# at-wat/mcl_3dl

Measured on AMD Instinct MI355X. Metric: particle·point evals/sec; filter-update Hz @ 4096 particles × 16k-pt scan, higher is better.
Workload: dtype f32

## Files before the change

### mcl_3dl_amd/csrc/host_measure.h

```cpp
#pragma once
#include <type_traits>

namespace
{
int ensure_structures(mcl3dl_hip_ctx* ctx, bool need_lik, bool need_dda, bool need_cells = false)
{
  if (!ctx->has_map)
    return ctx->fail(-5, "no map: call mcl3dl_hip_set_map first");
  bool built = false;
  if (need_lik && ctx->opt.lik_index == 0 && !need_cells && !ctx->lik_params_set && (ctx->lik_cell_from_beam || lik_cell_is_beams(ctx)))
  {
    ctx->lik_params_set = true;
    if (ctx->lik_cell_from_beam)
      ctx->lik_dirty = ctx->lik_base_dirty = true;
  }
  if (need_lik && (ctx->opt.lik_index == 0 || need_cells) && ctx->lik_dirty)
  {
    TRY(build_lik_grid(ctx));
    built = true;
  }
  if (need_lik && ctx->opt.lik_index == 0 && !need_cells)
  {
    const int dim[3] = { ctx->lg.nx, ctx->lg.ny, ctx->lg.nz };
    if (!lik_scan_provable(dim))
// ... 26 lines not shown
  k.r2_sq = static_cast<float>(static_cast<double>(r2) * static_cast<double>(r2));
  const double cell = 1.0 / static_cast<double>(ctx->lg.inv_cell);
  const auto reach = [&](float r) { return static_cast<int>(std::min(std::ceil(static_cast<double>(r) / cell + 0.005), 1.0e6)); };
  k.reach1 = reach(r1);
  k.reach2 = reach(r2);
  k.wx = ctx->weight[0];
  k.wy = ctx->weight[1];
  k.wz = ctx->weight[2];
  k.has_weight = ctx->has_weight ? 1 : 0;
  k.map = ctx->map_dev.as<float4>();
  k.occ = ctx->kd_occ.as<uint32_t>();
  return k;
}

int ensure_caster_structures(mcl3dl_hip_ctx* ctx, bool need_lik, bool need_beam, bool need_cells = false)
{
  if (ctx->beam_raycast != 1)
    return ensure_structures(ctx, need_lik, need_beam, need_cells);
  TRY(ensure_structures(ctx, need_lik, false, need_cells));
  if (need_beam)
  {
    if (ctx->lik_dirty)
    {
      TRY(build_lik_grid(ctx));
      scratch_trim(ctx, 64u << 20);
    }
    TRY(ensure_map_dev(ctx));
    const KdRayParams k = kd_ray_params(ctx);
    if (ctx->kd_occ_reach != k.reach1)
    {
      const unsigned long long n_cells = static_cast<unsigned long long>(ctx->lg.nx) * ctx->lg.ny * ctx->lg.nz;
      const unsigned long long blocks = (n_cells + 255) / 256;
      if (blocks > 0x7fffffffull)
        return ctx->fail(-4, "the cell grid has too many cells for the kd-tree caster's occupancy bitmap");
      TRY(ensure(ctx, ctx->kd_occ, sizeof(unsigned long long) * ((n_cells + 63) / 64)));
      hipLaunchKernelGGL(kd_occupancy_kernel, dim3(static_cast<unsigned>(blocks)), dim3(256), 0, ctx->stream, ctx->lg, k.reach1,
                         n_cells, ctx->kd_occ.as<unsigned long long>());
      HIP_TRY(hipGetLastError());
      ctx->kd_occ_reach = k.reach1;
    }
  }
  return 0;
}

using HostOut = PfEmit;

LikParams lik_params(const mcl3dl_hip_ctx* ctx)
{
  LikParams p;
  p.wx = ctx->weight[0];
  p.wy = ctx->weight[1];
  p.wz = ctx->weight[2];
  p.has_weight = ctx->has_weight ? 1 : 0;
  p.match_dist_min = ctx->match_dist_min;
  p.r2 = static_cast<float>(static_cast<double>(ctx->match_dist_min) * static_cast<double>(ctx->match_dist_min));
  p.match_dist_flat = ctx->match_dist_flat;
  p.match_weight = ctx->match_weight;
  return p;
}

BeamParams beam_params(const mcl3dl_hip_ctx* ctx)
{
  BeamParams p;
  p.sin_total_ref = ctx->sin_total_ref;
  p.hit_range_sq = ctx->hit_range_sq;
  p.filter_label_max = ctx->filter_label_max;
  p.short_only = ctx->short_only;
  p.beam_likelihood_min = ctx->beam_likelihood_min;
  return p;
}

void beam_refresh(mcl3dl_hip_ctx* ctx)
{
  ctx->hit_range_sq = static_cast<float>(std::pow(static_cast<double>(ctx->hit_range), 2));
  ctx->beam_likelihood = static_cast<float>(
      std::pow(static_cast<double>(ctx->beam_likelihood_min), 1.0 / static_cast<float>(ctx->beam_num_points)));
  ctx->sin_total_ref = sinf(ctx->ang_total_ref);
  ctx->pow_table_dirty = true;
}

uint64_t morton3(uint32_t x, uint32_t y, uint32_t z)
{
  auto spread = [](uint64_t v)
  {
    v &= 0x1fffff;
    v = (v | v << 32) & 0x1f00000000ffffULL;
    v = (v | v << 16) & 0x1f0000ff0000ffULL;
    v = (v | v << 8) & 0x100f00f00f00f00fULL;
    v = (v | v << 4) & 0x10c30c30c30c30c3ULL;
    v = (v | v << 2) & 0x1249249249249249ULL;
    return v;
  };
  return spread(x) | (spread(y) << 1) | (spread(z) << 2);
}

int ensure_pow_table(mcl3dl_hip_ctx* ctx, size_t n_b_coming = 0)
{
  const size_t n_b = std::max(ctx->n_b, n_b_coming);
  if (!(ctx->pow_table_dirty || n_b > ctx->pow_table_len))
    return 0;
  const size_t len = std::max<size_t>(n_b, 1024);
  std::vector<float> table(len + 1);
  table[0] = 1.0f;
  for (size_t k = 1; k <= len; ++k)
    table[k] = table[k - 1] * ctx->beam_likelihood;
  TRY(ensure(ctx, ctx->pow_table, sizeof(float) * table.size()));
// ... 969 lines not shown
```

### mcl_3dl_amd/csrc/likelihood_kernels.h

```cpp
#pragma once
#include <hip/hip_runtime.h>
#include <stdint.h>

#include "device_math.h"
#include "float_chain.h"
#include "map_structs.h"
#pragma clang fp contract(off)

namespace mcl3dl
{
template <bool STATS>
__device__ inline float nearest_d2(const LikGrid& g, float qx, float qy, float qz, unsigned& n_tested)
{
  const float fx = floorf((qx - g.ox) * g.inv_cell);
  const float fy = floorf((qy - g.oy) * g.inv_cell);
  const float fz = floorf((qz - g.oz) * g.inv_cell);
  float best = 3.0e38f;
  if (!(fx >= 1.0f && fy >= 1.0f && fz >= 1.0f && fx <= static_cast<float>(g.nx - 2) &&
        fy <= static_cast<float>(g.ny - 2) && fz <= static_cast<float>(g.nz - 2)))
    return best;
  const int cx = static_cast<int>(fx), cy = static_cast<int>(fy), cz = static_cast<int>(fz);
  uint32_t rs[9], re[9];
#pragma unroll
  for (int r = 0; r < 9; ++r)
  {
    const int dz = r / 3 - 1, dy = r % 3 - 1;
    const size_t row = (static_cast<size_t>(cz + dz) * g.ny + (cy + dy)) * g.nx + cx;
    rs[r] = g.cell_start[row - 1];
    re[r] = g.cell_start[row + 2];
  }
#pragma unroll
  for (int r = 0; r < 9; ++r)
  {
    for (uint32_t k = rs[r]; k < re[r]; ++k)
    {
      const float4 p = g.pts[k];
      const float dx = qx - p.x, dy = qy - p.y, dz = qz - p.z;
      float d2 = dx * dx;
      d2 = d2 + dy * dy;
      d2 = d2 + dz * dz;
      best = d2 < best ? d2 : best;
      if (STATS)
        ++n_tested;
    }
  }
  return best;
}

__device__ inline float d2_simple(float qx, float qy, float qz, float px, float py, float pz)
{
  const float dx = qx - px, dy = qy - py, dz = qz - pz;
  float d2 = dx * dx;
  d2 = d2 + dy * dy;
  d2 = d2 + dz * dz;
  return d2;
}

__global__ void radius_search_kernel(const float* __restrict__ query_xyz, int n, LikGrid g, LikParams prm, float radius,
                                     float r2, int reach, int* __restrict__ out_index, float* __restrict__ out_sqdist)
// ... 552 lines not shown
  {
    __shared__ float s_small[256];
    const int row = static_cast<int>(threadIdx.x) - i;
    if (i < n_s)
      s_small[row + static_cast<int>(perm[i])] = term;
    __syncthreads();
    float s = 0.0f;
    if (i == 0)
      for (int j = 0; j < n_s; ++j)
        s = s + s_small[row + j];
    lik = s;
  }
  else
  {
    double acc = static_cast<double>(term);
#pragma unroll
    for (int off = W / 2; off > 0; off >>= 1)
      acc += __shfl_down(acc, off, W);
    lik = static_cast<float>(acc);
  }
#pragma unroll
  for (int off = W / 2; off > 0; off >>= 1)
    num += __shfl_down(num, off, W);
  if (i == 0 && p < n_p)
  {
    if (out_lik)
      out_lik[p] = lik;
    if (out_ratio)
      out_ratio[p] = static_cast<float>(num) / static_cast<float>(n_s);
  }
}

struct LikChain
{
  unsigned long long* carry;
  uint32_t tag0;
  float* out_lik;
  float* out_ratio;
  float* also_fill;
  volatile unsigned* err;
};

__device__ inline unsigned long long chain_pack(uint32_t value, uint32_t tag)
{
  return (static_cast<unsigned long long>(tag) << 32) | value;
}

template <bool B>
struct BoolConstant
{
  static constexpr bool value = B;
};

constexpr int DEFER_QCAP = 96;

struct DeferQueue
{
  uint32_t word[4][DEFER_QCAP];
  uint16_t who[4][DEFER_QCAP];
};

template <bool FAST = false>
__device__ inline float eval_coop_first(const RecGrid& rg, const LikParams& prm, const Vec3f pos, const Quat rot, const float4 v,
                                        bool have_point, int lane, bool& matched, bool& over, float& best, uint32_t& mine,
                                        unsigned long long& over_m, unsigned long long* matched_m = nullptr)
{
  const Vec3f tp = vadd(qrot_trim(rot, Vec3f{ v.x, v.y, v.z }), pos);
  const float qx = tp.x * prm.wx, qy = tp.y * prm.wy, qz = tp.z * prm.wz;
  uint32_t ti, sub;
  const bool inside = rec_locate<FAST>(rg, qx, qy, qz, ti, sub) && have_point;
  int b;
  if constexpr (FAST)
  {
    const unsigned long long base = reinterpret_cast<unsigned long long>(rg.brick_table);
    const u32x4 tb = { static_cast<uint32_t>(base), (static_cast<uint32_t>(base >> 32) & 0xffffu) | (4u << 16), rg.table_bytes32,
                       0x00020000u };
    asm volatile("buffer_load_dword %0, %1, %2, 0 idxen\n\ts_waitcnt vmcnt(0)" : "=v"(b) : "v"(inside ? ti : rg.ti_empty), "s"(tb) : "memory");
  }
  else
    b = rg.brick_table[inside ? ti : rg.ti_empty];
  const bool valid = b >= 0;
  float dist = -1.0f;
  over = false;
  over_m = 0ull;
  best = 0.0f;
  mine = 0u;
  const unsigned long long valid_m = __builtin_amdgcn_ballot_w64(valid);
  if (valid_m != 0ull)
  {
    if constexpr (FAST)
      asm("" : "+v"(sub));
    uint32_t rec = (static_cast<uint32_t>(b) << 9) | sub;
    if constexpr (FAST)
      asm("" : "+v"(rec));
    const uint32_t vrec = (FAST || rg.rec_bytes32) ? rec : (valid ? rec : 0u);
    uint32_t w[4];
    best = quad_round<FAST>(rg.rec, rg.rec_bytes32, vrec, qx, qy, qz, lane & 3, w);
    mine = own_word(w, lane & 3);
    over_m = valid_m & lanes_gt_u32(mine, rg.over_thr);
    if (rg.bound_step > 0.0f && over_m != 0ull)
    {
      asm volatile("");
      over_m &= __builtin_amdgcn_fcmpf(best, rec_bound2(rg, mine), 2 );
    }
    over = __builtin_amdgcn_inverse_ballot_w64(over_m);
    if constexpr (FAST)
    {
      const unsigned long long in_m = valid_m & ~over_m & __builtin_amdgcn_fcmpf(best, prm.r2, 4 );
      float out = over ? best : 0.0f * prm.match_weight;
      if (__builtin_amdgcn_inverse_ballot_w64(in_m))
        out = lik_dist(prm, sqrt_in_radius(best)) * prm.match_weight;
      *matched_m = in_m;
      matched = __builtin_amdgcn_inverse_ballot_w64(in_m);
      return out;
    }
    if (valid && !over && best < prm.r2)
    {
      const float s = sqrt_in_radius(best);
      dist = lik_dist(prm, s);
    }
  }
  if constexpr (FAST)
  {
    *matched_m = 0ull;
    matched = false;
    return 0.0f * prm.match_weight;
  }
  matched = !(dist < 0.0f);
  return lik_term(prm, dist, matched);
}

template <bool FAST = false, int G, int LD>
__device__ inline void defer_drain(const RecGrid& rg, const LikParams& prm, const float (&s_pose)[G][8], float (&s_term)[G][LD],
                                   unsigned (&s_cnt)[G][4], const DeferQueue& q, int wave, int lane, uint32_t base, uint32_t n,
                                   const float4 v)
{
  __builtin_amdgcn_fence(__ATOMIC_RELEASE, "wavefront");
  __builtin_amdgcn_wave_barrier();
  const bool act = static_cast<uint32_t>(lane) < n;
  const uint32_t slot = act ? base + static_cast<uint32_t>(lane) : base;
  const uint32_t word = q.word[wave][slot];
  const uint32_t who = q.who[wave][slot];
  const int src = static_cast<int>(who & 63u), k = static_cast<int>(who >> 6);
  const Vec3f pt = { __shfl(v.x, src), __shfl(v.y, src), __shfl(v.z, src) };
  const Vec3f pos = { s_pose[k][0], s_pose[k][1], s_pose[k][2] };
  const Quat rot = { s_pose[k][3], s_pose[k][4], s_pose[k][5], s_pose[k][6] };
  const Vec3f tp = vadd(qrot_trim(rot, pt), pos);
  const float qx = tp.x * prm.wx, qy = tp.y * prm.wy, qz = tp.z * prm.wz;
  const int t_src = wave * 64 + src;
  float best = s_term[k][t_src];
  const uint32_t ext = word & rec_ext_mask(rg);
  const uint32_t rounds = act ? rec_overflow_records(word >> rg.count_shift, 4u, rg.count_is_records) : 0u;
  for (uint32_t r = 0; wave_any(r < rounds); ++r)
  {
    const bool more = r < rounds;
    uint32_t unused[4];
    const float m = quad_round<FAST>(rg.ovf, rg.ovf_bytes32, more ? ext + r : 0u, qx, qy, qz, lane & 3, unused);
    best = (more && m < best) ? m : best;
  }
  if constexpr (FAST)
  {
    if (act)
    {
      const bool in = best < prm.r2;
      s_term[k][t_src] = in ? lik_dist(prm, sqrt_in_radius(best)) * prm.match_weight : 0.0f * prm.match_weight;
      if (in)
        atomicAdd(&s_cnt[k][wave], 1u);
    }
    return;
  }
  float dist = -1.0f;
  if (act && best < prm.r2)
  {
    const float s = sqrt_in_radius(best);
    dist = lik_dist(prm, s);
  }
  if (act)
  {
    s_term[k][t_src] = lik_term(prm, dist, !(dist < 0.0f));
    if (!(dist < 0.0f))
      atomicAdd(&s_cnt[k][wave], 1u);
  }
}

template <bool FAST, int G, int LD>
__device__ __forceinline__ uint32_t defer_push(const RecGrid& rg, const LikParams& prm, const float (&s_pose)[G][8],
                                               float (&s_term)[G][LD], unsigned (&s_cnt)[G][4], DeferQueue& q, int wave, int lane,
                                               const float4 v, uint32_t qn, unsigned long long over_m, bool over, uint32_t mine,
                                               int k)
{
  if (over_m != 0ull)
  {
    const uint32_t n_new = static_cast<uint32_t>(__popcll(over_m));
    if (qn + n_new > static_cast<uint32_t>(DEFER_QCAP))
    {
      defer_drain<FAST>(rg, prm, s_pose, s_term, s_cnt, q, wave, lane, 0u, qn, v);
      qn = 0;
    }
    if (over)
    {
      const uint32_t slot = qn + __builtin_amdgcn_mbcnt_hi(static_cast<uint32_t>(over_m >> 32),
                                                           __builtin_amdgcn_mbcnt_lo(static_cast<uint32_t>(over_m), 0u));
      q.word[wave][slot] = mine;
      q.who[wave][slot] = static_cast<uint16_t>((static_cast<uint32_t>(k) << 6) | static_cast<uint32_t>(lane));
    }
    qn += n_new;
    if (qn >= 64u)
    {
      defer_drain<FAST>(rg, prm, s_pose, s_term, s_cnt, q, wave, lane, qn - 64u, 64u, v);
      qn -= 64u;
    }
  }
  return qn;
}

template <bool FAST, int G, int LD>
__device__ __forceinline__ void defer_flush(const RecGrid& rg, const LikParams& prm, const float (&s_pose)[G][8],
                                            float (&s_term)[G][LD], unsigned (&s_cnt)[G][4], const DeferQueue& q, int wave,
                                            int lane, const float4 v, uint32_t qn)
{
  defer_drain<FAST>(rg, prm, s_pose, s_term, s_cnt, q, wave, lane, 0u, qn, v);
}

template <int G>
__device__ __forceinline__ void stage_poses(float (&s_pose)[G][8], const float* __restrict__ pose7, int n_p, int group, int t)
{
  if (t < G)
  {
    const int p = group * G + t;
    float valid = 0.f;
    if (p < n_p)
    {
      const float* ps = pose7 + 7 * static_cast<size_t>(p);
      const Quat r = qnormalized(Quat{ ps[3], ps[4], ps[5], ps[6] });
      s_pose[t][0] = ps[0];
      s_pose[t][1] = ps[1];
      s_pose[t][2] = ps[2];
      s_pose[t][3] = r.x;
      s_pose[t][4] = r.y;
      s_pose[t][5] = r.z;
      s_pose[t][6] = r.w;
      valid = 1.f;
    }
    s_pose[t][7] = valid;
  }
}

__device__ __forceinline__ bool xcd_row_map(uint32_t block_index, int n_groups, int n_links, int& link, int& group)
{
  const uint32_t xcd = block_index & 7u, seq = block_index >> 3, ng = static_cast<uint32_t>(n_groups);
  const uint32_t row = seq / ng;
  link = static_cast<int>(row * 8u + xcd);
  group = static_cast<int>(seq - row * ng);
  return link < n_links;
}

constexpr int CHAIN_POLL_MAX = 1 << 20;
__device__ __forceinline__ void chain_take(const LikChain& ch, const unsigned long long* cw, int link, float& s,
                                           uint32_t& cnt)
{
  s = 0.0f;
  cnt = 0;
  if (link > 0)
  {
    const uint32_t want = ch.tag0 + static_cast<uint32_t>(link) - 1u;
    unsigned long long a = 0, b = 0;
#pragma nounroll
    for (int polls = 0;; ++polls)
    {
      a = __hip_atomic_load(cw, __ATOMIC_RELAXED, __HIP_MEMORY_SCOPE_AGENT);
      b = __hip_atomic_load(cw + 1, __ATOMIC_RELAXED, __HIP_MEMORY_SCOPE_AGENT);
      if (static_cast<uint32_t>(a >> 32) == want && static_cast<uint32_t>(b >> 32) == want)
        break;
      if (polls >= CHAIN_POLL_MAX)
// ... 33 lines not shown
    if (ch.also_fill)
      ch.also_fill[p] = 1.0f;
  }
  else
  {
    const uint32_t tag = ch.tag0 + static_cast<uint32_t>(link);
    __hip_atomic_store(cw, chain_pack(__float_as_uint(s), tag), __ATOMIC_RELAXED, __HIP_MEMORY_SCOPE_AGENT);
    __hip_atomic_store(cw + 1, chain_pack(cnt, tag), __ATOMIC_RELAXED, __HIP_MEMORY_SCOPE_AGENT);
  }
}

template <int G, int MODE, int MINW = 8, bool COOP = false, bool DEFER = false, bool CHAIN = false>
__device__ __forceinline__ void likelihood_tiled_body(const uint32_t block_index, const float* __restrict__ pose7, int n_p,
                                                      const float4* __restrict__ scan, int n_s, int n_tiles, int n_groups,
                                                      LikGrid g, RecGrid rg, LikParams prm,
                                                      double* __restrict__ partial_sum, unsigned* __restrict__ partial_cnt,
                                                      const uint32_t* __restrict__ scan_perm, float* __restrict__ strict_terms,
                                                      int strict_skew4, LikChain ch)
{
  constexpr int TERM_LD = CHAIN ? 260 : 256;
  __shared__ __attribute__((aligned(16))) float s_pose[G][8];
  __shared__ __attribute__((aligned(16))) float s_term[G][TERM_LD];
  __shared__ unsigned s_cnt[G][4];
  const uint32_t xcd = block_index & 7u;
  const uint32_t seq = block_index >> 3;
  const uint32_t ng = static_cast<uint32_t>(n_groups);
  const uint32_t full_tiles = static_cast<uint32_t>(n_tiles) & ~7u;
  const uint32_t per_xcd_full = (full_tiles >> 3) * ng;
  int tile, group;
  if constexpr (CHAIN)
  {
    if (!xcd_row_map(block_index, n_groups, n_tiles, tile, group))
      return;
  }
  else if (seq < per_xcd_full)
  {
    const uint32_t row = seq / ng;
    tile = static_cast<int>(row * 8u + xcd);
    group = static_cast<int>(seq - row * ng);
  }
  else
  {
    const uint32_t rem_items = (static_cast<uint32_t>(n_tiles) - full_tiles) * ng;
    const uint32_t per_xcd_rem = (rem_items + 7u) >> 3;
    const uint32_t s2 = seq - per_xcd_full;
    const uint32_t item = xcd * per_xcd_rem + s2;
    if (s2 >= per_xcd_rem || item >= rem_items)
      return;
    const uint32_t row = item / ng;
    tile = static_cast<int>(full_tiles + row);
    group = static_cast<int>(item - row * ng);
  }
  const int t = threadIdx.x, lane = t & 63, wave = t >> 6;
  stage_poses<G>(s_pose, pose7, n_p, group, t);
  const int i = tile * 256 + t;
  const bool have_point = i < n_s;
  const float4 v = have_point ? scan[i] : make_float4(0.f, 0.f, 0.f, 0.f);
  __syncthreads();
  const int n_valid = min(G, n_p - group * G);
  if constexpr (COOP && MODE == 2 && DEFER)
  {
    __shared__ DeferQueue s_q;
    const auto pose_loop = [&](auto fast) {
      constexpr bool FAST = decltype(fast)::value;
      uint32_t qn = 0;
      typedef float f32x4 __attribute__((ext_vector_type(4)));
      typedef __attribute__((address_space(3))) const f32x4 LdsPose;
      typedef __attribute__((address_space(3))) float LdsTerm;
      typedef __attribute__((address_space(3))) unsigned LdsCount;
      LdsPose* p_pose = (LdsPose*)&s_pose[0][0];
      LdsTerm* p_term = (LdsTerm*)&s_term[0][t];
      LdsCount* p_cnt = (LdsCount*)&s_cnt[0][wave];
      for (int k = 0; k < n_valid; ++k)
      {
        LdsPose* ps = FAST ? p_pose : (LdsPose*)&s_pose[k][0];
        const f32x4 pa = ps[0], pb = ps[1];
        const Vec3f pos = { pa.x, pa.y, pa.z };
        const Quat rot = { pa.w, pb.x, pb.y, pb.z };
        bool matched, over;
        float best;
        uint32_t mine;
        unsigned long long om;
        unsigned long long m;
        if constexpr (FAST)
        {
          *p_term = eval_coop_first<true>(rg, prm, pos, rot, v, have_point, lane, matched, over, best, mine, om, &m);
          if (lane == 0)
            *p_cnt = static_cast<unsigned>(__popcll(m));
          asm volatile("" : "+v"(p_pose), "+v"(p_term), "+v"(p_cnt));
          p_pose += 2;
          p_term += TERM_LD;
          p_cnt += 4;
        }
        else
        {
          const float term = eval_coop_first(rg, prm, pos, rot, v, have_point, lane, matched, over, best, mine, om);
          s_term[k][t] = over ? best : term;
          m = __builtin_amdgcn_ballot_w64(matched);
          if (lane == 0)
            s_cnt[k][wave] = static_cast<unsigned>(__popcll(m));
        }
        qn = defer_push<FAST>(rg, prm, s_pose, s_term, s_cnt, s_q, wave, lane, v, qn, om, over, mine, k);
      }
      if (qn != 0u)
        defer_flush<FAST>(rg, prm, s_pose, s_term, s_cnt, s_q, wave, lane, v, qn);
    };
    if (rg.common_map)
      pose_loop(BoolConstant<true>{});
    else
      pose_loop(BoolConstant<false>{});
  }
  else if constexpr (COOP && MODE == 2)
  {
    for (int k = 0; k < n_valid; ++k)
    {
      const Vec3f pos = { s_pose[k][0], s_pose[k][1], s_pose[k][2] };
      const Quat rot = { s_pose[k][3], s_pose[k][4], s_pose[k][5], s_pose[k][6] };
      bool matched;
      const float term = eval_coop(rg, prm, pos, rot, v, have_point, lane, matched);
      s_term[k][t] = term;
      const unsigned long long m = __builtin_amdgcn_ballot_w64(matched);
      if (lane == 0)
        s_cnt[k][wave] = static_cast<unsigned>(__popcll(m));
    }
  }
  else
  for (int k = 0; k < n_valid; ++k)
  {
    const Vec3f pos = { s_pose[k][0], s_pose[k][1], s_pose[k][2] };
    const Quat rot = { s_pose[k][3], s_pose[k][4], s_pose[k][5], s_pose[k][6] };
    float term = 0.f;
    bool matched = false;
    if (have_point)
    {
      const Vec3f tp = vadd(qrot(rot, Vec3f{ v.x, v.y, v.z }), pos);
      const float qx = tp.x * prm.wx, qy = tp.y * prm.wy, qz = tp.z * prm.wz;
      unsigned dummy = 0;
      const float d2 = MODE == 0 ? nearest_d2<false>(g, qx, qy, qz, dummy) :
                                   nearest_d2_rec<false>(rg, qx, qy, qz, dummy);
      if (d2 < prm.r2)
      {
        const float s = sqrtf(d2);
        const float dist = prm.match_dist_min - (s > prm.match_dist_flat ? s : prm.match_dist_flat);
        if (!(dist < 0.0f))
        {
          term = dist * prm.match_weight;
          matched = true;
        }
      }
    }
    s_term[k][t] = term;
    const unsigned long long m = __ballot(matched);
    if (lane == 0)
      s_cnt[k][wave] = static_cast<unsigned>(__popcll(m));
  }
  __syncthreads();
  if constexpr (CHAIN)
  {
    if (wave != 0 || lane >= n_valid)
      return;
    const int k = lane;
    const size_t p = static_cast<size_t>(group) * G + k;
    unsigned long long* cw = ch.carry + 2 * p;
    float s;
    uint32_t cnt;
    chain_take(ch, cw, tile, s, cnt);
    chain_add_row(&s_term[k][0], s);
    cnt += s_cnt[k][0] + s_cnt[k][1] + s_cnt[k][2] + s_cnt[k][3];
    chain_give(ch, cw, p, tile, tile == n_tiles - 1, n_s, s, cnt);
    return;
  }
  if (strict_terms)
  {
    constexpr int Q = G / 4;
    float4* rows = reinterpret_cast<float4*>(strict_terms) + static_cast<size_t>(group) * (static_cast<size_t>(n_s) * Q + strict_skew4);
#pragma unroll
    for (int j = 0; j < Q; ++j)
    {
      const int e = t + 256 * j, pt = e / Q, k4 = (e % Q) * 4;
      const int src = tile * 256 + pt;
      if (src < n_s)
        rows[static_cast<size_t>(scan_perm[src]) * Q + (e % Q)] =
            make_float4(s_term[k4][pt], s_term[k4 + 1][pt], s_term[k4 + 2][pt], s_term[k4 + 3][pt]);
    }
  }
  constexpr int LPP = 256 / G;
  constexpr int SEG = 256 / LPP;
  const int pk = t / LPP, seg = t % LPP;
  double acc = 0.0;
  if (pk < n_valid)
  {
#pragma unroll 8
    for (int j = 0; j < SEG; ++j)
    {
      const int jj = (j + t) % SEG;
      acc += static_cast<double>(s_term[pk][seg * SEG + jj]);
    }
  }
#pragma unroll
  for (int off = LPP / 2; off > 0; off >>= 1)
    acc += __shfl_down(acc, off, LPP);
  if (seg == 0 && pk < n_valid)
  {
    const size_t o = static_cast<size_t>(tile) * n_p + (group * G + pk);
    partial_sum[o] = acc;
    partial_cnt[o] = s_cnt[pk][0] + s_cnt[pk][1] + s_cnt[pk][2] + s_cnt[pk][3];
  }
}

template <int G, int MODE, int MINW = 8, bool COOP = false, bool DEFER = false, bool CHAIN = false>
__global__ __launch_bounds__(256, MINW) void likelihood_tiled_kernel(const float* __restrict__ pose7, int n_p,
                                                               const float4* __restrict__ scan, int n_s, int n_tiles,
                                                               int n_groups, LikGrid g, RecGrid rg,
                                                               LikParams prm, double* __restrict__ partial_sum,
                                                               unsigned* __restrict__ partial_cnt,
                                                               const uint32_t* __restrict__ scan_perm,
                                                               float* __restrict__ strict_terms, int strict_skew4 = 0,
                                                               LikChain ch = LikChain{})
{
  likelihood_tiled_body<G, MODE, MINW, COOP, DEFER, CHAIN>(blockIdx.x, pose7, n_p, scan, n_s, n_tiles, n_groups, g, rg, prm, partial_sum,
                                                           partial_cnt, scan_perm, strict_terms, strict_skew4, ch);
}

__global__ __launch_bounds__(256) void lik_finalize_kernel(const double* __restrict__ partial_sum,
                                                           const unsigned* __restrict__ partial_cnt, int n_tiles, int n_p,
                                                           int n_s, float* __restrict__ out_lik,
                                                           float* __restrict__ out_ratio, float* __restrict__ also_fill)
{
  __shared__ double s_a[8][32];
  __shared__ unsigned s_n[8][32];
  const int pl = threadIdx.x & 31, slice = threadIdx.x >> 5;
  const int p = blockIdx.x * 32 + pl;
  double a = 0.0;
  unsigned n = 0;
  if (p < n_p)
  {
    for (int tl = slice; tl < n_tiles; tl += 8)
    {
      a += partial_sum[static_cast<size_t>(tl) * n_p + p];
      n += partial_cnt[static_cast<size_t>(tl) * n_p + p];
    }
  }
  s_a[slice][pl] = a;
// ... 172 lines not shown
```

### mcl_3dl_amd/csrc/map_structs.h

```cpp
#pragma once
#include <hip/hip_runtime.h>
#include <stdint.h>

#include "device_math.h"
#include "map_compiler.h"
#pragma clang fp contract(off)

namespace mcl3dl
{
struct LikGrid
{
  const uint32_t* cell_start;
  const float4* pts;
  float ox, oy, oz;
  float inv_cell;
  int nx, ny, nz;
};

struct LikParams
{
  float wx, wy, wz;
  int has_weight;
  float match_dist_min;
  float r2;
  float match_dist_flat;
  float match_weight;
};

struct DdaGrid
{
  const unsigned long long* bricks;
  int bnx, bny, bnz;
  int mul24_ok;
  const uint32_t* vox_start;
  const float4* pts;
  const uint32_t* pt_index;
  const uint32_t* ov_key;
  const float4* ov_pts;
  const uint32_t* ov_idx;
  int ov_n;
  uint32_t ov_base;
  float min_x, min_y, min_z;
  float max_x, max_y, max_z;
  int nx, ny, nz;
  double grid;
  double ray_angle_half;
  double min_dist_thr_sq;
  float hit_tolerance_f;
};

struct BeamParams
{
  float sin_total_ref;
  float hit_range_sq;
  uint32_t filter_label_max;
  int short_only;
  float beam_likelihood_min;
};

}
```

### mcl_3dl_amd/csrc/pf_kernels.h

```cpp
#pragma once
#include <hip/hip_runtime.h>
#include <stdint.h>

#include "device_math.h"
#include "float_chain.h"
#include "motion_kernels.h"

#pragma clang fp contract(off)

namespace mcl3dl
{
constexpr int PF_BLOCK = 256;

struct PfEmit
{
  float* stats4;
  float* w;
  float* lik;
  float* ratio;
  float* beam;
};

struct BeamCounts
{
// ... 34 lines not shown
    const float wn = w[i] * l;
    w_new[i] = wn;
    s += static_cast<double>(wn);
    if (wn > 0.0f)
      t += static_cast<double>(wn) * log(static_cast<double>(wn));
    if (ratio)
    {
      const double r = static_cast<double>(ratio[i]);
      rmax = r > rmax ? r : rmax;
      rneg = -r > rneg ? -r : rneg;
    }
  }
  __shared__ double sh[4][PF_BLOCK / 64];
  s = wave_sum(s);
  t = wave_sum(t);
  rmax = wave_max(rmax);
  rneg = wave_max(rneg);
  const int lane = threadIdx.x & 63, wave = threadIdx.x >> 6;
  if (lane == 0)
  {
    sh[0][wave] = s;
    sh[1][wave] = t;
    sh[2][wave] = rmax;
    sh[3][wave] = rneg;
  }
  __syncthreads();
  if (threadIdx.x == 0)
  {
    double a = 0, b = 0, c = sh[2][0], d = sh[3][0];
    for (int k = 0; k < PF_BLOCK / 64; ++k)
    {
      a += sh[0][k];
      b += sh[1][k];
      c = sh[2][k] > c ? sh[2][k] : c;
      d = sh[3][k] > d ? sh[3][k] : d;
    }
    block_partials[4 * blockIdx.x + 0] = a;
    block_partials[4 * blockIdx.x + 1] = b;
    block_partials[4 * blockIdx.x + 2] = c;
    block_partials[4 * blockIdx.x + 3] = d;
  }
}

struct LikTiles
{
  const double* psum;
  const unsigned* pcnt;
  int n_tiles, n_s;
  float* lik_out;
  float* ratio_out;
  float* beam_fill;
  BeamCounts bc;
};
__global__ __launch_bounds__(256) void lik_pf_partial_kernel(LikTiles lt, const float* __restrict__ w,
                                                             const float* __restrict__ beam, const float* __restrict__ extra,
                                                             int n, float* __restrict__ w_new,
                                                             double* __restrict__ wave_partials)
{
  __shared__ double s_a[8][64];
  __shared__ unsigned s_n[8][64];
  const int lane = threadIdx.x & 63, wave = threadIdx.x >> 6;
  const int p = blockIdx.x * 64 + lane;
  double a0 = 0.0, a1 = 0.0;
  unsigned n0 = 0, n1 = 0;
  if (p < n)
  {
    const double* ps = lt.psum + p;
    const unsigned* pc = lt.pcnt + p;
    int tl = wave;
    for (; tl + 4 < lt.n_tiles; tl += 8)
    {
      const double x0 = ps[static_cast<size_t>(tl) * n], x1 = ps[static_cast<size_t>(tl + 4) * n];
      const unsigned c0 = pc[static_cast<size_t>(tl) * n], c1 = pc[static_cast<size_t>(tl + 4) * n];
      a0 += x0;
      a1 += x1;
      n0 += c0;
      n1 += c1;
    }
    if (tl < lt.n_tiles)
    {
      a0 += ps[static_cast<size_t>(tl) * n];
      n0 += pc[static_cast<size_t>(tl) * n];
    }
  }
  s_a[wave][lane] = a0;
  s_a[wave + 4][lane] = a1;
  s_n[wave][lane] = n0;
  s_n[wave + 4][lane] = n1;
  __syncthreads();
  if (wave != 0)
    return;
  double s = 0.0, t = 0.0, rmax = 0.0, rneg = -1.0;
  if (p < n)
  {
    double a = a0;
    unsigned cnt = n0;
#pragma unroll
    for (int k = 1; k < 8; ++k)
    {
      a += s_a[k][lane];
      cnt += s_n[k][lane];
    }
    const float lk = static_cast<float>(a);
    const float r32 = static_cast<float>(cnt) / static_cast<float>(lt.n_s);
    lt.lik_out[p] = lk;
    lt.ratio_out[p] = r32;
    if (lt.beam_fill)
      lt.beam_fill[p] = 1.0f;
    float l = 1.0f;
    if (lt.bc.penalty)
      l *= beam_score_from_count(lt.bc, p);
    else if (beam)
      l *= lt.beam_fill ? 1.0f : beam[p];
    l *= lk;
    if (extra)
      l = l * extra[p];
    const float wn = w[p] * l;
    w_new[p] = wn;
    s += static_cast<double>(wn);
    if (wn > 0.0f)
      t += static_cast<double>(wn) * log(static_cast<double>(wn));
    const double r = static_cast<double>(r32);
    rmax = r > rmax ? r : rmax;
    rneg = -r > rneg ? -r : rneg;
  }
  s = wave_sum(s);
  t = wave_sum(t);
  rmax = wave_max(rmax);
  rneg = wave_max(rneg);
  if (lane == 0)
  {
    wave_partials[4 * blockIdx.x + 0] = s;
    wave_partials[4 * blockIdx.x + 1] = t;
    wave_partials[4 * blockIdx.x + 2] = rmax;
    wave_partials[4 * blockIdx.x + 3] = rneg;
  }
}

__device__ inline void pf_reduce_lanes(const double* __restrict__ block_partials, int n_blocks, int n_waves, int lane, double& a,
                                       double& b, double& c, double& d)
{
  a = 0;
  b = 0;
  c = 0.0;
  d = -1.0;
  if (n_waves > 0)
  {
    for (int k = lane; k < n_blocks; k += 64)
    {
      const double* wp = block_partials + 16 * static_cast<size_t>(k);
      const bool h1 = 4 * k + 1 < n_waves, h2 = 4 * k + 2 < n_waves, h3 = 4 * k + 3 < n_waves;
      double ba = 0, bb = 0, bc = wp[2], bd = wp[3];
      ba += wp[0];
      bb += wp[1];
      const double a1 = h1 ? wp[4] : 0.0, b1 = h1 ? wp[5] : 0.0, c1 = h1 ? wp[6] : 0.0, d1 = h1 ? wp[7] : -1.0;
      const double a2 = h2 ? wp[8] : 0.0, b2 = h2 ? wp[9] : 0.0, c2 = h2 ? wp[10] : 0.0, d2 = h2 ? wp[11] : -1.0;
      const double a3 = h3 ? wp[12] : 0.0, b3 = h3 ? wp[13] : 0.0, c3 = h3 ? wp[14] : 0.0, d3 = h3 ? wp[15] : -1.0;
      ba += a1;
      bb += b1;
      bc = c1 > bc ? c1 : bc;
      bd = d1 > bd ? d1 : bd;
      ba += a2;
      bb += b2;
      bc = c2 > bc ? c2 : bc;
      bd = d2 > bd ? d2 : bd;
      ba += a3;
      bb += b3;
      bc = c3 > bc ? c3 : bc;
      bd = d3 > bd ? d3 : bd;
      a += ba;
      b += bb;
      c = bc > c ? bc : c;
      d = bd > d ? bd : d;
    }
  }
  else
  for (int k = lane; k < n_blocks; k += 64)
  {
    a += block_partials[4 * k + 0];
    b += block_partials[4 * k + 1];
    c = block_partials[4 * k + 2] > c ? block_partials[4 * k + 2] : c;
    d = block_partials[4 * k + 3] > d ? block_partials[4 * k + 3] : d;
  }
  a = wave_sum(a);
  b = wave_sum(b);
  c = wave_max(c);
  d = wave_max(d);
}

__global__ __launch_bounds__(64) void pf_reduce_kernel(const double* __restrict__ block_partials, int n_blocks, int rank,
                                                       int world, double* __restrict__ packed, int n_waves = 0)
{
  double a, b, c, d;
  pf_reduce_lanes(block_partials, n_blocks, n_waves, threadIdx.x, a, b, c, d);
  if (threadIdx.x == 0)
  {
    packed[0] = a;
    packed[1] = b;
    for (int r = 0; r < world; ++r)
    {
      packed[2 + 2 * r] = (r == rank) ? c : 0.0;
      packed[3 + 2 * r] = (r == rank) ? d : 0.0;
    }
  }
}

__global__ __launch_bounds__(PF_BLOCK) void pf_apply_kernel(float* __restrict__ w, const float* __restrict__ w_new,
                                                            int n, int world, const double* __restrict__ packed_in,
                                                            float* __restrict__ stats4, PfEmit emit = PfEmit{},
                                                            const float* __restrict__ lik = nullptr,
                                                            const float* __restrict__ ratio = nullptr,
                                                            const float* __restrict__ beam = nullptr,
                                                            const double* __restrict__ partials = nullptr, int n_blocks = 0,
                                                            int n_waves = 0, double* __restrict__ packed_w = nullptr)
{
  __shared__ double s_tot[4];
  const double* packed = packed_in;
  if (partials)
  {
    if (threadIdx.x < 64)
    {
      double a, b, c, d;
      pf_reduce_lanes(partials, n_blocks, n_waves, threadIdx.x, a, b, c, d);
      if (threadIdx.x == 0)
      {
        s_tot[0] = a;
        s_tot[1] = b;
        s_tot[2] = c;
        s_tot[3] = d;
        if (blockIdx.x == 0 && packed_w)
        {
          packed_w[0] = a;
          packed_w[1] = b;
          packed_w[2] = c;
          packed_w[3] = d;
        }
      }
    }
    __syncthreads();
    packed = s_tot;
  }
  const double S = packed[0];
  const float sum_f = static_cast<float>(S);
  const bool alive = sum_f > 0.0f;
  if (alive)
  {
    for (int i = blockIdx.x * PF_BLOCK + threadIdx.x; i < n; i += gridDim.x * PF_BLOCK)
    {
      const float wv = w_new[i] / sum_f;
      w[i] = wv;
      if (emit.w)
        emit.w[i] = wv;
    }
  }
  else if (emit.w)
  {
    for (int i = blockIdx.x * PF_BLOCK + threadIdx.x; i < n; i += gridDim.x * PF_BLOCK)
      emit.w[i] = w[i];
  }
  if (emit.lik || emit.ratio || emit.beam)
    for (int i = blockIdx.x * PF_BLOCK + threadIdx.x; i < n; i += gridDim.x * PF_BLOCK)
    {
      if (emit.lik)
        emit.lik[i] = lik[i];
      if (emit.ratio)
        emit.ratio[i] = ratio[i];
      if (emit.beam)
        emit.beam[i] = beam[i];
    }
  if (blockIdx.x == 0 && threadIdx.x == 0 && (stats4 || emit.stats4))
  {
    double rmax = packed[2], rneg = packed[3];
    for (int r = 1; r < world; ++r)
    {
      rmax = packed[2 + 2 * r] > rmax ? packed[2 + 2 * r] : rmax;
      rneg = packed[3 + 2 * r] > rneg ? packed[3 + 2 * r] : rneg;
    }
    const float st[4] = { alive ? static_cast<float>(log(S) - packed[1] / S) : __builtin_nanf(""), static_cast<float>(-rneg),
                          static_cast<float>(rmax), alive ? 0.0f : 1.0f };
    for (int k = 0; k < 4; ++k)
    {
      if (stats4)
        stats4[k] = st[k];
      if (emit.stats4)
        emit.stats4[k] = st[k];
    }
  }
}

constexpr int PF_FUSED_MAX = 4096;

__global__ __launch_bounds__(1024) void pf_fused_kernel(float* __restrict__ w, const float* __restrict__ lik,
                                                        const float* __restrict__ beam, const float* __restrict__ extra,
                                                        const float* __restrict__ ratio, int n, float* __restrict__ w_new,
                                                        double* __restrict__ packed, float* __restrict__ stats4,
                                                        PfEmit emit = PfEmit{}, int float_order = 0, BeamCounts bc = BeamCounts{},
                                                        ImuGravity imu = ImuGravity{})
{
  __shared__ __attribute__((aligned(16))) float s_w[PF_FUSED_MAX + 4];
  __shared__ double sh[4][16];
  __shared__ double part[4][16];
  __shared__ double tot[4];
  const int nb = (n + PF_BLOCK - 1) / PF_BLOCK;
  const int q = threadIdx.x >> 8, tid = threadIdx.x & 255, lane = threadIdx.x & 63, wave = threadIdx.x >> 6;
  for (int vb0 = 0; vb0 < nb; vb0 += 4)
  {
    const int vb = vb0 + q;
    double s = 0.0, t = 0.0, rmax = 0.0, rneg = -1.0;
    const int i = vb * PF_BLOCK + tid;
    if (vb < nb && i < n)
    {
      float l = 1.0f;
      if (bc.penalty)
        l *= beam_score_from_count(bc, i);
      else if (beam)
        l *= beam[i];
      l *= imu.state13 ? imu_gravity_likelihood(imu, i) : lik[i];
      if (extra)
        l = l * extra[i];
      const float wn = w[i] * l;
      w_new[i] = wn;
// ... 474 lines not shown
```

Measured before the change: 306.6 billion.

## Specialize unit-weight queries, permute LDS term slots, prefetch PF reduction inputs

Adds a compile-time specialization that skips the per-axis weight multiply when the map weights are unity. It also permutes the shared-memory term layout so the per-pose reduction can read float4 chunks with XOR-swizzled bank mapping instead of a scalar strided loop. The particle-filter partial kernel now issues all per-tile partial-sum loads in an unrolled batch when the tile count is small, and both PF kernels prefetch per-particle inputs early to hide latency. These are several independent changes that add template instantiations and code size, and the slot permutation must stay consistent between every writer and reader.

Measured after the change: 315.3 billion (median of 6 runs). +2.9%, better.

```diff
diff --git a/mcl_3dl_amd/csrc/host_measure.h b/mcl_3dl_amd/csrc/host_measure.h
--- a/mcl_3dl_amd/csrc/host_measure.h
+++ b/mcl_3dl_amd/csrc/host_measure.h
@@ -102,6 +102,7 @@
   p.wy = ctx->weight[1];
   p.wz = ctx->weight[2];
   p.has_weight = ctx->has_weight ? 1 : 0;
+  p.unit_form = lik_unit_form(p.wx, p.wy, p.wz);
   p.match_dist_min = ctx->match_dist_min;
   p.r2 = static_cast<float>(static_cast<double>(ctx->match_dist_min) * static_cast<double>(ctx->match_dist_min));
   p.match_dist_flat = ctx->match_dist_flat;
diff --git a/mcl_3dl_amd/csrc/likelihood_kernels.h b/mcl_3dl_amd/csrc/likelihood_kernels.h
--- a/mcl_3dl_amd/csrc/likelihood_kernels.h
+++ b/mcl_3dl_amd/csrc/likelihood_kernels.h
@@ -5,6 +5,7 @@
 #include "device_math.h"
 #include "float_chain.h"
 #include "map_structs.h"
+#include "term_slots.h"
 #pragma clang fp contract(off)
 
 namespace mcl3dl
@@ -663,6 +664,12 @@
   static constexpr bool value = B;
 };
 
+template <int I>
+struct IntConstant
+{
+  static constexpr int value = I;
+};
+
 constexpr int DEFER_QCAP = 96;
 
 struct DeferQueue
@@ -671,13 +678,13 @@
   uint16_t who[4][DEFER_QCAP];
 };
 
-template <bool FAST = false>
+template <bool FAST = false, int WFORM = 0>
 __device__ inline float eval_coop_first(const RecGrid& rg, const LikParams& prm, const Vec3f pos, const Quat rot, const float4 v,
                                         bool have_point, int lane, bool& matched, bool& over, float& best, uint32_t& mine,
                                         unsigned long long& over_m, unsigned long long* matched_m = nullptr)
 {
   const Vec3f tp = vadd(qrot_trim(rot, Vec3f{ v.x, v.y, v.z }), pos);
-  const float qx = tp.x * prm.wx, qy = tp.y * prm.wy, qz = tp.z * prm.wz;
+  const float qx = WFORM >= 1 ? tp.x : tp.x * prm.wx, qy = WFORM >= 1 ? tp.y : tp.y * prm.wy, qz = WFORM >= 2 ? tp.z : tp.z * prm.wz;
   uint32_t ti, sub;
   const bool inside = rec_locate<FAST>(rg, qx, qy, qz, ti, sub) && have_point;
   int b;
@@ -741,7 +748,7 @@
   return lik_term(prm, dist, matched);
 }
 
-template <bool FAST = false, int G, int LD>
+template <bool FAST = false, int WFORM = 0, int G, int LD>
 __device__ inline void defer_drain(const RecGrid& rg, const LikParams& prm, const float (&s_pose)[G][8], float (&s_term)[G][LD],
                                    unsigned (&s_cnt)[G][4], const DeferQueue& q, int wave, int lane, uint32_t base, uint32_t n,
                                    const float4 v)
@@ -757,8 +764,8 @@
   const Vec3f pos = { s_pose[k][0], s_pose[k][1], s_pose[k][2] };
   const Quat rot = { s_pose[k][3], s_pose[k][4], s_pose[k][5], s_pose[k][6] };
   const Vec3f tp = vadd(qrot_trim(rot, pt), pos);
-  const float qx = tp.x * prm.wx, qy = tp.y * prm.wy, qz = tp.z * prm.wz;
-  const int t_src = wave * 64 + src;
+  const float qx = WFORM >= 1 ? tp.x : tp.x * prm.wx, qy = WFORM >= 1 ? tp.y : tp.y * prm.wy, qz = WFORM >= 2 ? tp.z : tp.z * prm.wz;
+  const int t_src = term_slot<G, LD != 256>(wave * 64 + src);
   float best = s_term[k][t_src];
   const uint32_t ext = word & rec_ext_mask(rg);
   const uint32_t rounds = act ? rec_overflow_records(word >> rg.count_shift, 4u, rg.count_is_records) : 0u;
@@ -794,7 +801,7 @@
   }
 }
 
-template <bool FAST, int G, int LD>
+template <bool FAST, int WFORM = 0, int G, int LD>
 __device__ __forceinline__ uint32_t defer_push(const RecGrid& rg, const LikParams& prm, const float (&s_pose)[G][8],
                                                float (&s_term)[G][LD], unsigned (&s_cnt)[G][4], DeferQueue& q, int wave, int lane,
                                                const float4 v, uint32_t qn, unsigned long long over_m, bool over, uint32_t mine,
@@ -805,7 +812,7 @@
     const uint32_t n_new = static_cast<uint32_t>(__popcll(over_m));
     if (qn + n_new > static_cast<uint32_t>(DEFER_QCAP))
     {
-      defer_drain<FAST>(rg, prm, s_pose, s_term, s_cnt, q, wave, lane, 0u, qn, v);
+      defer_drain<FAST, WFORM>(rg, prm, s_pose, s_term, s_cnt, q, wave, lane, 0u, qn, v);
       qn = 0;
     }
     if (over)
@@ -818,19 +825,19 @@
     qn += n_new;
     if (qn >= 64u)
     {
-      defer_drain<FAST>(rg, prm, s_pose, s_term, s_cnt, q, wave, lane, qn - 64u, 64u, v);
+      defer_drain<FAST, WFORM>(rg, prm, s_pose, s_term, s_cnt, q, wave, lane, qn - 64u, 64u, v);
       qn -= 64u;
     }
   }
   return qn;
 }
 
-template <bool FAST, int G, int LD>
+template <bool FAST, int WFORM = 0, int G, int LD>
 __device__ __forceinline__ void defer_flush(const RecGrid& rg, const LikParams& prm, const float (&s_pose)[G][8],
                                             float (&s_term)[G][LD], unsigned (&s_cnt)[G][4], const DeferQueue& q, int wave,
                                             int lane, const float4 v, uint32_t qn)
 {
-  defer_drain<FAST>(rg, prm, s_pose, s_term, s_cnt, q, wave, lane, 0u, qn, v);
+  defer_drain<FAST, WFORM>(rg, prm, s_pose, s_term, s_cnt, q, wave, lane, 0u, qn, v);
 }
 
 template <int G>
@@ -970,6 +977,7 @@
     group = static_cast<int>(item - row * ng);
   }
   const int t = threadIdx.x, lane = t & 63, wave = t >> 6;
+  const int tslot = term_slot<G, CHAIN>(t);
   stage_poses<G>(s_pose, pose7, n_p, group, t);
   const int i = tile * 256 + t;
   const bool have_point = i < n_s;
@@ -979,15 +987,16 @@
   if constexpr (COOP && MODE == 2 && DEFER)
   {
     __shared__ DeferQueue s_q;
-    const auto pose_loop = [&](auto fast) {
+    const auto pose_loop = [&](auto fast, auto wform) {
       constexpr bool FAST = decltype(fast)::value;
+      constexpr int WFORM = decltype(wform)::value;
       uint32_t qn = 0;
       typedef float f32x4 __attribute__((ext_vector_type(4)));
       typedef __attribute__((address_space(3))) const f32x4 LdsPose;
       typedef __attribute__((address_space(3))) float LdsTerm;
       typedef __attribute__((address_space(3))) unsigned LdsCount;
       LdsPose* p_pose = (LdsPose*)&s_pose[0][0];
-      LdsTerm* p_term = (LdsTerm*)&s_term[0][t];
+      LdsTerm* p_term = (LdsTerm*)&s_term[0][tslot];
       LdsCount* p_cnt = (LdsCount*)&s_cnt[0][wave];
       for (int k = 0; k < n_valid; ++k)
       {
@@ -1002,7 +1011,7 @@
         unsigned long long m;
         if constexpr (FAST)
         {
-          *p_term = eval_coop_first<true>(rg, prm, pos, rot, v, have_point, lane, matched, over, best, mine, om, &m);
+          *p_term = eval_coop_first<true, WFORM>(rg, prm, pos, rot, v, have_point, lane, matched, over, best, mine, om, &m);
           if (lane == 0)
             *p_cnt = static_cast<unsigned>(__popcll(m));
           asm volatile("" : "+v"(p_pose), "+v"(p_term), "+v"(p_cnt));
@@ -1013,20 +1022,24 @@
         else
         {
           const float term = eval_coop_first(rg, prm, pos, rot, v, have_point, lane, matched, over, best, mine, om);
-          s_term[k][t] = over ? best : term;
+          s_term[k][tslot] = over ? best : term;
           m = __builtin_amdgcn_ballot_w64(matched);
           if (lane == 0)
             s_cnt[k][wave] = static_cast<unsigned>(__popcll(m));
         }
-        qn = defer_push<FAST>(rg, prm, s_pose, s_term, s_cnt, s_q, wave, lane, v, qn, om, over, mine, k);
+        qn = defer_push<FAST, WFORM>(rg, prm, s_pose, s_term, s_cnt, s_q, wave, lane, v, qn, om, over, mine, k);
       }
       if (qn != 0u)
-        defer_flush<FAST>(rg, prm, s_pose, s_term, s_cnt, s_q, wave, lane, v, qn);
+        defer_flush<FAST, WFORM>(rg, prm, s_pose, s_term, s_cnt, s_q, wave, lane, v, qn);
     };
-    if (rg.common_map)
-      pose_loop(BoolConstant<true>{});
+    if (!rg.common_map)
+      pose_loop(BoolConstant<false>{}, IntConstant<0>{});
+    else if (prm.unit_form == 2)
+      pose_loop(BoolConstant<true>{}, IntConstant<2>{});
+    else if (prm.unit_form == 1)
+      pose_loop(BoolConstant<true>{}, IntConstant<1>{});
     else
-      pose_loop(BoolConstant<false>{});
+      pose_loop(BoolConstant<true>{}, IntConstant<0>{});
   }
   else if constexpr (COOP && MODE == 2)
   {
@@ -1036,7 +1049,7 @@
       const Quat rot = { s_pose[k][3], s_pose[k][4], s_pose[k][5], s_pose[k][6] };
       bool matched;
       const float term = eval_coop(rg, prm, pos, rot, v, have_point, lane, matched);
-      s_term[k][t] = term;
+      s_term[k][tslot] = term;
       const unsigned long long m = __builtin_amdgcn_ballot_w64(matched);
       if (lane == 0)
         s_cnt[k][wave] = static_cast<unsigned>(__popcll(m));
@@ -1067,7 +1080,7 @@
         }
       }
     }
-    s_term[k][t] = term;
+    s_term[k][tslot] = term;
     const unsigned long long m = __ballot(matched);
     if (lane == 0)
       s_cnt[k][wave] = static_cast<unsigned>(__popcll(m));
@@ -1096,17 +1109,34 @@
     for (int j = 0; j < Q; ++j)
     {
       const int e = t + 256 * j, pt = e / Q, k4 = (e % Q) * 4;
-      const int src = tile * 256 + pt;
+      const int src = tile * 256 + pt, sl = term_slot<G, CHAIN>(pt);
       if (src < n_s)
         rows[static_cast<size_t>(scan_perm[src]) * Q + (e % Q)] =
-            make_float4(s_term[k4][pt], s_term[k4 + 1][pt], s_term[k4 + 2][pt], s_term[k4 + 3][pt]);
+            make_float4(s_term[k4][sl], s_term[k4 + 1][sl], s_term[k4 + 2][sl], s_term[k4 + 3][sl]);
     }
   }
   constexpr int LPP = 256 / G;
   constexpr int SEG = 256 / LPP;
   const int pk = t / LPP, seg = t % LPP;
   double acc = 0.0;
-  if (pk < n_valid)
+  if constexpr (TermSlots<G, CHAIN>::permuted)
+  {
+    if (pk < n_valid)
+    {
+      const float4* row = reinterpret_cast<const float4*>(&s_term[pk][0]);
+      const int first = (seg * (SEG / 4)) ^ term_chunk_xor<G>(seg);
+#pragma unroll
+      for (int c = 0; c < SEG / 4; ++c)
+      {
+        const float4 q = row[first ^ c];
+        acc += static_cast<double>(q.x);
+        acc += static_cast<double>(q.y);
+        acc += static_cast<double>(q.z);
+        acc += static_cast<double>(q.w);
+      }
+    }
+  }
+  else if (pk < n_valid)
   {
 #pragma unroll 8
     for (int j = 0; j < SEG; ++j)
diff --git a/mcl_3dl_amd/csrc/map_structs.h b/mcl_3dl_amd/csrc/map_structs.h
--- a/mcl_3dl_amd/csrc/map_structs.h
+++ b/mcl_3dl_amd/csrc/map_structs.h
@@ -21,11 +21,17 @@
 {
   float wx, wy, wz;
   int has_weight;
+  int unit_form;
   float match_dist_min;
   float r2;
   float match_dist_flat;
   float match_weight;
 };
+
+__host__ __device__ inline int lik_unit_form(float wx, float wy, float wz)
+{
+  return (wx == 1.0f && wy == 1.0f) ? (wz == 1.0f ? 2 : 1) : 0;
+}
 
 struct DdaGrid
 {
diff --git a/mcl_3dl_amd/csrc/pf_kernels.h b/mcl_3dl_amd/csrc/pf_kernels.h
--- a/mcl_3dl_amd/csrc/pf_kernels.h
+++ b/mcl_3dl_amd/csrc/pf_kernels.h
@@ -110,6 +110,7 @@
   float* beam_fill;
   BeamCounts bc;
 };
+constexpr int LIK_TAIL_UNROLL = 16;
 __global__ __launch_bounds__(256) void lik_pf_partial_kernel(LikTiles lt, const float* __restrict__ w,
                                                              const float* __restrict__ beam, const float* __restrict__ extra,
                                                              int n, float* __restrict__ w_new,
@@ -119,26 +120,60 @@
   __shared__ unsigned s_n[8][64];
   const int lane = threadIdx.x & 63, wave = threadIdx.x >> 6;
   const int p = blockIdx.x * 64 + lane;
+  const bool read_beam = !lt.bc.penalty && beam && !lt.beam_fill;
+  float w_p = 0.0f, beam_p = 1.0f, extra_p = 1.0f;
+  if (wave == 0 && p < n)
+  {
+    w_p = w[p];
+    if (read_beam)
+      beam_p = beam[p];
+    if (extra)
+      extra_p = extra[p];
+  }
   double a0 = 0.0, a1 = 0.0;
   unsigned n0 = 0, n1 = 0;
   if (p < n)
   {
     const double* ps = lt.psum + p;
     const unsigned* pc = lt.pcnt + p;
-    int tl = wave;
-    for (; tl + 4 < lt.n_tiles; tl += 8)
-    {
-      const double x0 = ps[static_cast<size_t>(tl) * n], x1 = ps[static_cast<size_t>(tl + 4) * n];
-      const unsigned c0 = pc[static_cast<size_t>(tl) * n], c1 = pc[static_cast<size_t>(tl + 4) * n];
-      a0 += x0;
-      a1 += x1;
-      n0 += c0;
-      n1 += c1;
-    }
-    if (tl < lt.n_tiles)
-    {
-      a0 += ps[static_cast<size_t>(tl) * n];
-      n0 += pc[static_cast<size_t>(tl) * n];
+    if (lt.n_tiles > 0 && lt.n_tiles <= 4 * LIK_TAIL_UNROLL)
+    {
+      double x[LIK_TAIL_UNROLL];
+      unsigned c[LIK_TAIL_UNROLL];
+#pragma unroll
+      for (int j = 0; j < LIK_TAIL_UNROLL; ++j)
+      {
+        const int tl = min(wave + 4 * j, lt.n_tiles - 1);
+        x[j] = ps[static_cast<size_t>(tl) * n];
+        c[j] = pc[static_cast<size_t>(tl) * n];
+      }
+#pragma unroll
+      for (int j = 0; j < LIK_TAIL_UNROLL; j += 2)
+      {
+        const bool h0 = wave + 4 * j < lt.n_tiles, h1 = wave + 4 * j + 4 < lt.n_tiles;
+        a0 = h0 ? a0 + x[j] : a0;
+        n0 = h0 ? n0 + c[j] : n0;
+        a1 = h1 ? a1 + x[j + 1] : a1;
+        n1 = h1 ? n1 + c[j + 1] : n1;
+      }
+    }
+    else
+    {
+      int tl = wave;
+      for (; tl + 4 < lt.n_tiles; tl += 8)
+      {
+        const double x0 = ps[static_cast<size_t>(tl) * n], x1 = ps[static_cast<size_t>(tl + 4) * n];
+        const unsigned c0 = pc[static_cast<size_t>(tl) * n], c1 = pc[static_cast<size_t>(tl + 4) * n];
+        a0 += x0;
+        a1 += x1;
+        n0 += c0;
+        n1 += c1;
+      }
+      if (tl < lt.n_tiles)
+      {
+        a0 += ps[static_cast<size_t>(tl) * n];
+        n0 += pc[static_cast<size_t>(tl) * n];
+      }
     }
   }
   s_a[wave][lane] = a0;
@@ -169,11 +204,11 @@
     if (lt.bc.penalty)
       l *= beam_score_from_count(lt.bc, p);
     else if (beam)
-      l *= lt.beam_fill ? 1.0f : beam[p];
+      l *= beam_p;
     l *= lk;
     if (extra)
-      l = l * extra[p];
-    const float wn = w[p] * l;
+      l = l * extra_p;
+    const float wn = w_p * l;
     w_new[p] = wn;
     s += static_cast<double>(wn);
     if (wn > 0.0f)
@@ -274,6 +309,19 @@
 {
   __shared__ double s_tot[4];
   const double* packed = packed_in;
+  const int i0 = blockIdx.x * PF_BLOCK + threadIdx.x;
+  const bool emits = emit.lik || emit.ratio || emit.beam;
+  float wn0 = 0.0f, lik0 = 0.0f, ratio0 = 0.0f, beam0 = 0.0f;
+  if (i0 < n)
+  {
+    wn0 = w_new[i0];
+    if (emit.lik)
+      lik0 = lik[i0];
+    if (emit.ratio)
+      ratio0 = ratio[i0];
+    if (emit.beam)
+      beam0 = beam[i0];
+  }
   if (partials)
   {
     if (threadIdx.x < 64)
@@ -303,9 +351,9 @@
   const bool alive = sum_f > 0.0f;
   if (alive)
   {
-    for (int i = blockIdx.x * PF_BLOCK + threadIdx.x; i < n; i += gridDim.x * PF_BLOCK)
-    {
-      const float wv = w_new[i] / sum_f;
+    for (int i = i0; i < n; i += gridDim.x * PF_BLOCK)
+    {
+      const float wv = (i == i0 ? wn0 : w_new[i]) / sum_f;
       w[i] = wv;
       if (emit.w)
         emit.w[i] = wv;
@@ -316,15 +364,15 @@
     for (int i = blockIdx.x * PF_BLOCK + threadIdx.x; i < n; i += gridDim.x * PF_BLOCK)
       emit.w[i] = w[i];
   }
-  if (emit.lik || emit.ratio || emit.beam)
-    for (int i = blockIdx.x * PF_BLOCK + threadIdx.x; i < n; i += gridDim.x * PF_BLOCK)
+  if (emits)
+    for (int i = i0; i < n; i += gridDim.x * PF_BLOCK)
     {
       if (emit.lik)
-        emit.lik[i] = lik[i];
+        emit.lik[i] = i == i0 ? lik0 : lik[i];
       if (emit.ratio)
-        emit.ratio[i] = ratio[i];
+        emit.ratio[i] = i == i0 ? ratio0 : ratio[i];
       if (emit.beam)
-        emit.beam[i] = beam[i];
+        emit.beam[i] = i == i0 ? beam0 : beam[i];
     }
   if (blockIdx.x == 0 && threadIdx.x == 0 && (stats4 || emit.stats4))
   {
diff --git a/mcl_3dl_amd/csrc/term_slots.h b/mcl_3dl_amd/csrc/term_slots.h
--- /dev/null
+++ b/mcl_3dl_amd/csrc/term_slots.h
@@ -0,0 +1,38 @@
+#pragma once
+
+#if defined(__HIPCC__)
+#define MCL3DL_SLOT_HD __host__ __device__
+#else
+#define MCL3DL_SLOT_HD
+#endif
+
+namespace mcl3dl
+{
+template <int G, bool CHAIN>
+struct TermSlots
+{
+  static constexpr bool permuted = !CHAIN && (G == 4 || G == 8 || G == 16);
+  static constexpr int SEG = G;
+};
+
+template <int G>
+MCL3DL_SLOT_HD constexpr int term_chunk_xor(int s)
+{
+  return G == 16 ? ((s >> 2) & 3) : G == 8 ? ((s >> 3) & 1) : 0;
+}
+
+template <int G, bool CHAIN>
+MCL3DL_SLOT_HD constexpr int term_slot(int i)
+{
+  if (!TermSlots<G, CHAIN>::permuted)
+    return i;
+  const int s = i / G, o = i % G;
+  return (s * G + ((o - s) & (G - 1))) ^ (term_chunk_xor<G>(s) << 2);
+}
+
+template <int G>
+MCL3DL_SLOT_HD constexpr int term_read_slot(int s, int j)
+{
+  return (s * G + j) ^ (term_chunk_xor<G>(s) << 2);
+}
+}
```
